# rishikksh20/FastSpeech2

Hardware: AMD Instinct MI355X
Metric: mel-frames/sec (higher is better)
Workload: dtype bf16x3 (FFN conv: f16 x f16 + block-scaled e4m3 cross terms; the decoder's: block-scaled e2m1 cross terms, one E8M0 scale per 16-channel block on both operands); 1 GPU; c3: batch=64 LJSpeech-shape; default.yaml dims, free-running, random-init weights (seed 0), duration bias calibrated to 7.87 frames/phoneme; precision=mix_mx4, utterances=64, phonemes=4528, parallelism=single GPU, launch=eager, device-driven layout (no host sync), overlap_encoder=False, streams=3

## Files before the change

fastspeech2_amd/csrc/attn_bf16.h:

```cpp
#pragma once
#include "common.h"
#include "gemm_bf16.h"

namespace fs2 {

constexpr int kAttAlign = 8;

struct QkvSplitArgs {
    const float* qkv; int R; int Rvt; int D; int dk; float scale;
    __bf16 *qk_hi, *qk_lo;
    __bf16 *vt_hi, *vt_lo;
};

__global__ __launch_bounds__(256) void qkv_split(QkvSplitArgs a) {
    extern __shared__ __attribute__((aligned(16))) float vt_s[];
    const int tid = threadIdx.x;
    const int r0 = blockIdx.x * 32;
    const int D = a.D, ld = 3 * D;
    const int groups = 2 * D / 8;
    for (int idx = tid; idx < 32 * groups; idx += 256) {
        const int r = idx / groups, c = (idx - r * groups) * 8;
        const int row = r0 + r;
        if (row >= a.R) continue;
        const float* src = a.qkv + (size_t)row * ld + c;
// ... 11 lines not shown
        const int r = idx / (D / 4), c = (idx - r * (D / 4)) * 4;
        const int row = r0 + r;
        float4 v = make_float4(0.f, 0.f, 0.f, 0.f);
        if (row < a.R) v = *reinterpret_cast<const float4*>(a.qkv + (size_t)row * ld + 2 * D + c);
        float* d = vt_s + r * ldv + c;
        d[0] = v.x; d[1] = v.y; d[2] = v.z; d[3] = v.w;
    }
    __syncthreads();
    for (int idx = tid; idx < D * 4; idx += 256) {
        const int n = idx >> 2, j = idx & 3;
        float4 p, q;
        const float* s = vt_s + (8 * j) * ldv + n;
        p.x = s[0]; p.y = s[ldv]; p.z = s[2 * ldv]; p.w = s[3 * ldv];
        q.x = s[4 * ldv]; q.y = s[5 * ldv]; q.z = s[6 * ldv]; q.w = s[7 * ldv];
        const SplitPair sp = split8(p, q);
        const size_t off = (size_t)n * a.Rvt + r0 + 8 * j;
        *reinterpret_cast<uint4*>(a.vt_hi + off) = sp.hi;
        *reinterpret_cast<uint4*>(a.vt_lo + off) = sp.lo;
    }
}

struct AttnB16Args {
    const __bf16 *qk_hi, *qk_lo; int ldqk;
    const __bf16 *vt_hi, *vt_lo; int Rvt;
    float* ctx; int ldc;
    void* ctxp; int ctxp_chunks;
    const int* start; const int* len; const int* klen;
    const int2* work;
    const int* nwork;
    int nitems;
    int D; int mask_q;
    unsigned qk_lo_bytes, vt_lo_bytes;
    int *slow_count, *slow_count2;
};

__device__ __forceinline__ float quad_rows_max(float v) {
    auto r = __builtin_amdgcn_permlane16_swap(__float_as_uint(v), __float_as_uint(v), false, false);
    v = fmaxf(__uint_as_float(r[0]), __uint_as_float(r[1]));
    r = __builtin_amdgcn_permlane32_swap(__float_as_uint(v), __float_as_uint(v), false, false);
    return fmaxf(__uint_as_float(r[0]), __uint_as_float(r[1]));
}
__device__ __forceinline__ float quad_rows_sum(float v) {
    auto r = __builtin_amdgcn_permlane16_swap(__float_as_uint(v), __float_as_uint(v), false, false);
    v = __uint_as_float(r[0]) + __uint_as_float(r[1]);
    r = __builtin_amdgcn_permlane32_swap(__float_as_uint(v), __float_as_uint(v), false, false);
    return __uint_as_float(r[0]) + __uint_as_float(r[1]);
}

template <int DK>
constexpr size_t attn_b16_lds_bytes() { return (size_t)32 * DK * 4 + (size_t)DK * 128; }

#ifdef FS2_ATT_TIMING
__device__ long long g_att_phase[8];
#define FS2_T(i) { const long long t_ = __builtin_readcyclecounter(); if (blockIdx.x == 0 && blockIdx.y == 0 && threadIdx.x == 0) g_att_phase[i] += t_ - tprev; tprev = t_; }
#else
#define FS2_T(i)
#endif

template <int DK, int NSPLIT>
__global__ __launch_bounds__(256, 2) void attn_bf16(AttnB16Args a) {
    extern __shared__ __attribute__((aligned(16))) char smem_a[];
    constexpr int KROW = DK * 4;
    constexpr int KSL = DK / 8;
    constexpr int NC = DK / 32;
    constexpr int NT = DK / 16;
    char* Ks = smem_a;
// ... 292 lines not shown
```

fastspeech2_amd/csrc/attn_w32.h:

```cpp
#pragma once
#include <type_traits>
#include <utility>
#include "attn_bf16.h"

namespace fs2 {

typedef float f32x16 __attribute__((ext_vector_type(16)));

template <int DK>
constexpr size_t attn_w32_lds_bytes() { return (size_t)3 * (32 * DK * 4 + DK * 128); }

template <class F, int... I>
__device__ __forceinline__ void for_seq(F&& f, std::integer_sequence<int, I...>) { (f(std::integral_constant<int, I>{}), ...); }

template <int N>
__device__ __forceinline__ void mfma_o0(const bf16x8_t& z_v) {
    if constexpr (N == 0) asm volatile("s_nop 3\n\tv_mfma_f32_32x32x16_bf16 a[0:15], %0, %0, 0" : : "v"(z_v) : "a0", "a1", "a2", "a3", "a4", "a5", "a6", "a7", "a8", "a9", "a10", "a11", "a12", "a13", "a14", "a15");
    else if constexpr (N == 1) asm volatile("s_nop 3\n\tv_mfma_f32_32x32x16_bf16 a[16:31], %0, %0, 0" : : "v"(z_v) : "a16", "a17", "a18", "a19", "a20", "a21", "a22", "a23", "a24", "a25", "a26", "a27", "a28", "a29", "a30", "a31");
    else if constexpr (N == 2) asm volatile("s_nop 3\n\tv_mfma_f32_32x32x16_bf16 a[32:47], %0, %0, 0" : : "v"(z_v) : "a32", "a33", "a34", "a35", "a36", "a37", "a38", "a39", "a40", "a41", "a42", "a43", "a44", "a45", "a46", "a47");
    else if constexpr (N == 3) asm volatile("s_nop 3\n\tv_mfma_f32_32x32x16_bf16 a[48:63], %0, %0, 0" : : "v"(z_v) : "a48", "a49", "a50", "a51", "a52", "a53", "a54", "a55", "a56", "a57", "a58", "a59", "a60", "a61", "a62", "a63");
    else if constexpr (N == 4) asm volatile("s_nop 3\n\tv_mfma_f32_32x32x16_bf16 a[64:79], %0, %0, 0" : : "v"(z_v) : "a64", "a65", "a66", "a67", "a68", "a69", "a70", "a71", "a72", "a73", "a74", "a75", "a76", "a77", "a78", "a79");
    else if constexpr (N == 5) asm volatile("s_nop 3\n\tv_mfma_f32_32x32x16_bf16 a[80:95], %0, %0, 0" : : "v"(z_v) : "a80", "a81", "a82", "a83", "a84", "a85", "a86", "a87", "a88", "a89", "a90", "a91", "a92", "a93", "a94", "a95");
    else if constexpr (N == 6) asm volatile("s_nop 3\n\tv_mfma_f32_32x32x16_bf16 a[96:111], %0, %0, 0" : : "v"(z_v) : "a96", "a97", "a98", "a99", "a100", "a101", "a102", "a103", "a104", "a105", "a106", "a107", "a108", "a109", "a110", "a111");
    else if constexpr (N == 7) asm volatile("s_nop 3\n\tv_mfma_f32_32x32x16_bf16 a[112:127], %0, %0, 0" : : "v"(z_v) : "a112", "a113", "a114", "a115", "a116", "a117", "a118", "a119", "a120", "a121", "a122", "a123", "a124", "a125", "a126", "a127");
}
template <int N>
__device__ __forceinline__ void read_o(float (&e)[16]) {
    if constexpr (N == 0) asm volatile("v_accvgpr_read_b32 %0, a0\n\tv_accvgpr_read_b32 %1, a1\n\tv_accvgpr_read_b32 %2, a2\n\tv_accvgpr_read_b32 %3, a3\n\tv_accvgpr_read_b32 %4, a4\n\tv_accvgpr_read_b32 %5, a5\n\tv_accvgpr_read_b32 %6, a6\n\tv_accvgpr_read_b32 %7, a7\n\tv_accvgpr_read_b32 %8, a8\n\tv_accvgpr_read_b32 %9, a9\n\tv_accvgpr_read_b32 %10, a10\n\tv_accvgpr_read_b32 %11, a11\n\tv_accvgpr_read_b32 %12, a12\n\tv_accvgpr_read_b32 %13, a13\n\tv_accvgpr_read_b32 %14, a14\n\tv_accvgpr_read_b32 %15, a15" : "=v"(e[0]), "=v"(e[1]), "=v"(e[2]), "=v"(e[3]), "=v"(e[4]), "=v"(e[5]), "=v"(e[6]), "=v"(e[7]), "=v"(e[8]), "=v"(e[9]), "=v"(e[10]), "=v"(e[11]), "=v"(e[12]), "=v"(e[13]), "=v"(e[14]), "=v"(e[15]));
    else if constexpr (N == 1) asm volatile("v_accvgpr_read_b32 %0, a16\n\tv_accvgpr_read_b32 %1, a17\n\tv_accvgpr_read_b32 %2, a18\n\tv_accvgpr_read_b32 %3, a19\n\tv_accvgpr_read_b32 %4, a20\n\tv_accvgpr_read_b32 %5, a21\n\tv_accvgpr_read_b32 %6, a22\n\tv_accvgpr_read_b32 %7, a23\n\tv_accvgpr_read_b32 %8, a24\n\tv_accvgpr_read_b32 %9, a25\n\tv_accvgpr_read_b32 %10, a26\n\tv_accvgpr_read_b32 %11, a27\n\tv_accvgpr_read_b32 %12, a28\n\tv_accvgpr_read_b32 %13, a29\n\tv_accvgpr_read_b32 %14, a30\n\tv_accvgpr_read_b32 %15, a31" : "=v"(e[0]), "=v"(e[1]), "=v"(e[2]), "=v"(e[3]), "=v"(e[4]), "=v"(e[5]), "=v"(e[6]), "=v"(e[7]), "=v"(e[8]), "=v"(e[9]), "=v"(e[10]), "=v"(e[11]), "=v"(e[12]), "=v"(e[13]), "=v"(e[14]), "=v"(e[15]));
    else if constexpr (N == 2) asm volatile("v_accvgpr_read_b32 %0, a32\n\tv_accvgpr_read_b32 %1, a33\n\tv_accvgpr_read_b32 %2, a34\n\tv_accvgpr_read_b32 %3, a35\n\tv_accvgpr_read_b32 %4, a36\n\tv_accvgpr_read_b32 %5, a37\n\tv_accvgpr_read_b32 %6, a38\n\tv_accvgpr_read_b32 %7, a39\n\tv_accvgpr_read_b32 %8, a40\n\tv_accvgpr_read_b32 %9, a41\n\tv_accvgpr_read_b32 %10, a42\n\tv_accvgpr_read_b32 %11, a43\n\tv_accvgpr_read_b32 %12, a44\n\tv_accvgpr_read_b32 %13, a45\n\tv_accvgpr_read_b32 %14, a46\n\tv_accvgpr_read_b32 %15, a47" : "=v"(e[0]), "=v"(e[1]), "=v"(e[2]), "=v"(e[3]), "=v"(e[4]), "=v"(e[5]), "=v"(e[6]), "=v"(e[7]), "=v"(e[8]), "=v"(e[9]), "=v"(e[10]), "=v"(e[11]), "=v"(e[12]), "=v"(e[13]), "=v"(e[14]), "=v"(e[15]));
    else if constexpr (N == 3) asm volatile("v_accvgpr_read_b32 %0, a48\n\tv_accvgpr_read_b32 %1, a49\n\tv_accvgpr_read_b32 %2, a50\n\tv_accvgpr_read_b32 %3, a51\n\tv_accvgpr_read_b32 %4, a52\n\tv_accvgpr_read_b32 %5, a53\n\tv_accvgpr_read_b32 %6, a54\n\tv_accvgpr_read_b32 %7, a55\n\tv_accvgpr_read_b32 %8, a56\n\tv_accvgpr_read_b32 %9, a57\n\tv_accvgpr_read_b32 %10, a58\n\tv_accvgpr_read_b32 %11, a59\n\tv_accvgpr_read_b32 %12, a60\n\tv_accvgpr_read_b32 %13, a61\n\tv_accvgpr_read_b32 %14, a62\n\tv_accvgpr_read_b32 %15, a63" : "=v"(e[0]), "=v"(e[1]), "=v"(e[2]), "=v"(e[3]), "=v"(e[4]), "=v"(e[5]), "=v"(e[6]), "=v"(e[7]), "=v"(e[8]), "=v"(e[9]), "=v"(e[10]), "=v"(e[11]), "=v"(e[12]), "=v"(e[13]), "=v"(e[14]), "=v"(e[15]));
    else if constexpr (N == 4) asm volatile("v_accvgpr_read_b32 %0, a64\n\tv_accvgpr_read_b32 %1, a65\n\tv_accvgpr_read_b32 %2, a66\n\tv_accvgpr_read_b32 %3, a67\n\tv_accvgpr_read_b32 %4, a68\n\tv_accvgpr_read_b32 %5, a69\n\tv_accvgpr_read_b32 %6, a70\n\tv_accvgpr_read_b32 %7, a71\n\tv_accvgpr_read_b32 %8, a72\n\tv_accvgpr_read_b32 %9, a73\n\tv_accvgpr_read_b32 %10, a74\n\tv_accvgpr_read_b32 %11, a75\n\tv_accvgpr_read_b32 %12, a76\n\tv_accvgpr_read_b32 %13, a77\n\tv_accvgpr_read_b32 %14, a78\n\tv_accvgpr_read_b32 %15, a79" : "=v"(e[0]), "=v"(e[1]), "=v"(e[2]), "=v"(e[3]), "=v"(e[4]), "=v"(e[5]), "=v"(e[6]), "=v"(e[7]), "=v"(e[8]), "=v"(e[9]), "=v"(e[10]), "=v"(e[11]), "=v"(e[12]), "=v"(e[13]), "=v"(e[14]), "=v"(e[15]));
    else if constexpr (N == 5) asm volatile("v_accvgpr_read_b32 %0, a80\n\tv_accvgpr_read_b32 %1, a81\n\tv_accvgpr_read_b32 %2, a82\n\tv_accvgpr_read_b32 %3, a83\n\tv_accvgpr_read_b32 %4, a84\n\tv_accvgpr_read_b32 %5, a85\n\tv_accvgpr_read_b32 %6, a86\n\tv_accvgpr_read_b32 %7, a87\n\tv_accvgpr_read_b32 %8, a88\n\tv_accvgpr_read_b32 %9, a89\n\tv_accvgpr_read_b32 %10, a90\n\tv_accvgpr_read_b32 %11, a91\n\tv_accvgpr_read_b32 %12, a92\n\tv_accvgpr_read_b32 %13, a93\n\tv_accvgpr_read_b32 %14, a94\n\tv_accvgpr_read_b32 %15, a95" : "=v"(e[0]), "=v"(e[1]), "=v"(e[2]), "=v"(e[3]), "=v"(e[4]), "=v"(e[5]), "=v"(e[6]), "=v"(e[7]), "=v"(e[8]), "=v"(e[9]), "=v"(e[10]), "=v"(e[11]), "=v"(e[12]), "=v"(e[13]), "=v"(e[14]), "=v"(e[15]));
    else if constexpr (N == 6) asm volatile("v_accvgpr_read_b32 %0, a96\n\tv_accvgpr_read_b32 %1, a97\n\tv_accvgpr_read_b32 %2, a98\n\tv_accvgpr_read_b32 %3, a99\n\tv_accvgpr_read_b32 %4, a100\n\tv_accvgpr_read_b32 %5, a101\n\tv_accvgpr_read_b32 %6, a102\n\tv_accvgpr_read_b32 %7, a103\n\tv_accvgpr_read_b32 %8, a104\n\tv_accvgpr_read_b32 %9, a105\n\tv_accvgpr_read_b32 %10, a106\n\tv_accvgpr_read_b32 %11, a107\n\tv_accvgpr_read_b32 %12, a108\n\tv_accvgpr_read_b32 %13, a109\n\tv_accvgpr_read_b32 %14, a110\n\tv_accvgpr_read_b32 %15, a111" : "=v"(e[0]), "=v"(e[1]), "=v"(e[2]), "=v"(e[3]), "=v"(e[4]), "=v"(e[5]), "=v"(e[6]), "=v"(e[7]), "=v"(e[8]), "=v"(e[9]), "=v"(e[10]), "=v"(e[11]), "=v"(e[12]), "=v"(e[13]), "=v"(e[14]), "=v"(e[15]));
    else if constexpr (N == 7) asm volatile("v_accvgpr_read_b32 %0, a112\n\tv_accvgpr_read_b32 %1, a113\n\tv_accvgpr_read_b32 %2, a114\n\tv_accvgpr_read_b32 %3, a115\n\tv_accvgpr_read_b32 %4, a116\n\tv_accvgpr_read_b32 %5, a117\n\tv_accvgpr_read_b32 %6, a118\n\tv_accvgpr_read_b32 %7, a119\n\tv_accvgpr_read_b32 %8, a120\n\tv_accvgpr_read_b32 %9, a121\n\tv_accvgpr_read_b32 %10, a122\n\tv_accvgpr_read_b32 %11, a123\n\tv_accvgpr_read_b32 %12, a124\n\tv_accvgpr_read_b32 %13, a125\n\tv_accvgpr_read_b32 %14, a126\n\tv_accvgpr_read_b32 %15, a127" : "=v"(e[0]), "=v"(e[1]), "=v"(e[2]), "=v"(e[3]), "=v"(e[4]), "=v"(e[5]), "=v"(e[6]), "=v"(e[7]), "=v"(e[8]), "=v"(e[9]), "=v"(e[10]), "=v"(e[11]), "=v"(e[12]), "=v"(e[13]), "=v"(e[14]), "=v"(e[15]));
}
template <int KIND>
__device__ __forceinline__ void mfma_s(f32x16& acc, const bf16x8_t& a_v, const bf16x8_t& b_a, const f32x16& cm) {
    if constexpr (KIND == 1) asm volatile("v_mfma_f32_32x32x16_bf16 %0, %1, %2, %3" : "=&v"(acc) : "v"(a_v), "a"(b_a), "v"(cm));
    else if constexpr (KIND == 2) asm volatile("v_mfma_f32_32x32x16_bf16 %0, %1, %2, 0" : "=&v"(acc) : "v"(a_v), "a"(b_a));
    else asm volatile("v_mfma_f32_32x32x16_bf16 %0, %1, %2, %0" : "+v"(acc) : "v"(a_v), "a"(b_a));
}
template <int N, bool PAD>
// ... 78 lines not shown
        const float p = __builtin_amdgcn_exp2f(score(key) - m);
        l += p;
#pragma unroll
        for (int c = 0; c < NC; ++c) acc[c] = fmaf(p, (float)vh[(size_t)c * a.Rvt + key] + (float)vl[(size_t)c * a.Rvt + key], acc[c]);
    }
    const float linv = (l > 0.f) ? 1.f / l : 0.f;
    const bool dead = a.mask_q && qrow >= klen;
    const size_t row = (size_t)(s0 + qrow);
#pragma unroll
    for (int c = 0; c < NC; c += 4) {
        const int col = h * DK + hi * NC + c;
        f32x4 v = f32x4{acc[c], acc[c + 1], acc[c + 2], acc[c + 3]} * linv;
        if (dead) v = f32x4{0.f, 0.f, 0.f, 0.f};
        if (a.ctx) *reinterpret_cast<f32x4*>(a.ctx + row * a.ldc + col) = v;
        if (a.ctxp) store_planes4(a.ctxp, row, a.ctxp_chunks, col, v);
    }
}

template <int DK>
__global__ __launch_bounds__(256, 1) void attn_w32(AttnB16Args a) {
    static_assert(DK % 64 == 0 && DK <= 256, "head dim: a multiple of 64 up to 256");
    extern __shared__ __attribute__((aligned(16))) char smem_w[];
    constexpr int KSL = DK / 8;
    constexpr int KROWB = DK * 4;
    constexpr int KB = 32 * KROWB;
    constexpr int VB = DK * 128;
    constexpr int NKS = DK / 16;
    constexpr int NT = DK / 32;
    constexpr int PW = DK / 32;
    using I0 = std::integral_constant<int, 0>;
    using I1 = std::integral_constant<int, 1>;
    const int tid = threadIdx.x, lane = tid & 63;
#ifdef FS2_W32_TIMING
    long long wstamp[12] = {0, 0, 0, 0, 0, 0, 0, 0, 0, 0, 0, 0};
    long long tpro = __builtin_readcyclecounter();
#define FS2_WP(i) { const long long t_ = __builtin_readcyclecounter(); wstamp[i] += t_ - tpro; tpro = t_; }
#else
#define FS2_WP(i)
#endif
    const int wave = __builtin_amdgcn_readfirstlane(tid >> 6);
    const int l31 = lane & 31, hi = lane >> 5;
    {
        const int nitems = a.nwork != nullptr ? *a.nwork : a.nitems;
        if ((int)blockIdx.x >= nitems) return;
    }
    const int2 wk = a.work[blockIdx.x];
    const int b = __builtin_amdgcn_readfirstlane(wk.x), h = blockIdx.y;
    if (b < 0) return;
    const int s0 = __builtin_amdgcn_readfirstlane(a.start[b]), len = __builtin_amdgcn_readfirstlane(a.len[b]);
    const int klen = __builtin_amdgcn_readfirstlane(a.klen[b]);
    const int q0 = __builtin_amdgcn_readfirstlane(wk.y) * kAttBlk + wave * 32;
    const bool wave_live = q0 < len;
    const int ntiles = (klen + 31) >> 5;
    const unsigned lds0 = __builtin_amdgcn_readfirstlane((unsigned)(size_t)(lds_void_t*)smem_w);
    FS2_WP(8)

    auto k_piece = [&](int u, int ln, int& key, int& byte_in_row) __attribute__((always_inline)) {
        const int G = (u * 4 + wave) * 64 + ln;
        const int rho = G / (2 * KSL), ps = G - rho * (2 * KSL);
        const int s = (ps & ~15) | ((ps & 15) ^ (rho & 15));
        const int plane = s >= KSL;
        key = (rho & 19) | ((rho & 4) << 1) | ((rho & 8) >> 1);
        byte_in_row = (s - plane * KSL) * 16 + plane * (int)a.qk_lo_bytes;
    };
    auto v_piece = [&](int u, int ln, int& n, int& j, int& plane) __attribute__((always_inline)) {
        const int G = (u * 4 + wave) * 64 + ln;
        n = G >> 3;
        const int s = (G & 7) ^ ((n >> 1) & 7);
        j = s & 3; plane = s >> 2;
    };
    unsigned kgo[PW], vgo[PW];
#pragma unroll
    for (int u = 0; u < PW; ++u) {
        int key, bir, n, j, plane;
        k_piece(u, lane, key, bir);
        kgo[u] = (unsigned)(key * a.ldqk * 2 + bir);
        v_piece(u, lane, n, j, plane);
        vgo[u] = (unsigned)n * (unsigned)a.Rvt * 2u + (unsigned)j * 16u + (unsigned)plane * a.vt_lo_bytes;
    }
    gchar_t* kbase = uniform_ptr(reinterpret_cast<const char*>(a.qk_hi + a.D + (size_t)h * DK) + (size_t)s0 * a.ldqk * 2);
    gchar_t* vbase = uniform_ptr(reinterpret_cast<const char*>(a.vt_hi + (size_t)h * DK * a.Rvt + s0));

    auto issue_K = [&](int kt, int buf) __attribute__((always_inline)) {
        const int key0 = kt * 32;
        const unsigned dst = lds0 + buf * KB + wave * 1024;
        if (key0 + 32 <= klen) {
            gchar_t* base = uniform_ptr((const void*)(kbase + (size_t)key0 * a.ldqk * 2));
            asm volatile("s_nop 4" ::: "memory");
#pragma unroll
            for (int u = 0; u < PW; ++u) dma16_so(base, kgo[u], dst + u * 4096);
        } else {
            int ln = lane;
            asm volatile("" : "+v"(ln));
#pragma unroll
            for (int u = 0; u < PW; ++u) {
                int key, bir;
                k_piece(u, ln, key, bir);
                dma16((const void*)(kbase + (size_t)min(key0 + key, klen - 1) * a.ldqk * 2 + bir), dst + u * 4096);
            }
        }
    };
    auto issue_V = [&](int kt, int buf) __attribute__((always_inline)) {
        const int key0 = kt * 32;
        const unsigned dst = lds0 + 3 * KB + buf * VB + wave * 1024;
        gchar_t* base = uniform_ptr((const void*)(vbase + (size_t)key0 * 2));
        if (key0 + 32 <= klen) {
            asm volatile("s_nop 4" ::: "memory");
#pragma unroll
            for (int u = 0; u < PW; ++u) dma16_so(base, vgo[u], dst + u * 4096);
        } else {
            int ln = lane;
            asm volatile("" : "+v"(ln));
#pragma unroll
            for (int u = 0; u < PW; ++u) {
                int n, j, plane;
                v_piece(u, ln, n, j, plane);
                const int nv = klen - (key0 + 8 * j);
                const unsigned go = (unsigned)n * (unsigned)a.Rvt * 2u + (unsigned)j * 16u + (unsigned)plane * a.vt_lo_bytes;
                const void* sp = (nv > 0) ? (const void*)(base + go) : static_cast<const void*>(g_zero16);
                dma16(sp, dst + u * 4096);
            }
        }
    };
    auto fix_V = [&](int kt, int buf) __attribute__((always_inline)) {
        const int key0 = kt * 32;
        if (key0 + 32 <= klen || (klen & 7) == 0) return;
        int ln = lane;
        asm volatile("" : "+v"(ln));
#pragma unroll
        for (int u = 0; u < PW; ++u) {
            int n, j, plane;
            v_piece(u, ln, n, j, plane);
            const int nv = klen - (key0 + 8 * j);
            if (nv > 0 && nv < 8) {
                u32x4* p = reinterpret_cast<u32x4*>(smem_w + 3 * KB + buf * VB + (u * 4 + wave) * 1024 + ln * 16);
                u32x4 v = *p;
#pragma unroll
                for (int w = 0; w < 4; ++w) v[w] &= (nv > 2 * w + 1) ? 0xffffffffu : ((nv > 2 * w) ? 0x0000ffffu : 0u);
                *p = v;
            }
        }
    };

    const char* kp[8];
    {
        const int g = hi ^ (l31 & 15);
#pragma unroll
        for (int e = 0; e < 8; ++e) kp[e] = smem_w + l31 * KROWB + ((((2 * e) ^ (g & 14)) | (g & 1)) << 4);
    }
    const char* vp[4];
    {
        const int g = hi ^ ((l31 >> 1) & 7);
#pragma unroll
        for (int e = 0; e < 4; ++e) vp[e] = smem_w + 3 * KB + l31 * 128 + ((((2 * e) ^ (g & 6)) | (g & 1)) << 4);
    }

    FS2_WP(9)
    if (ntiles > 0) issue_K(0, 0);
    static_assert(KB == VB, "the Q staging region spans K and V^T ring slots of equal size");
    bf16x8_t qh[NKS], ql[NKS];
    {
        gchar_t* qbase = (gchar_t*)reinterpret_cast<const char*>(a.qk_hi + (size_t)h * DK);
#pragma unroll
        for (int pc = 0; pc < KSL; ++pc) {
            const int G = pc * 64 + lane;
            const int rho = G / (2 * KSL), ps = G - rho * (2 * KSL);
            const int sl = (ps & ~15) | ((ps & 15) ^ (rho & 15));
            const int plane = sl >= KSL;
            const int qr = min(q0 + rho, len - 1);
            dma16((const void*)(qbase + (size_t)(s0 + qr) * a.ldqk * 2 + (sl - plane * KSL) * 16 + (size_t)plane * a.qk_lo_bytes), lds0 + (1 + wave) * KB + pc * 1024);
        }
        asm volatile("s_waitcnt vmcnt(0)" ::: "memory");
        const int qoff = (1 + wave) * KB;
#pragma unroll
        for (int c = 0; c < NKS; ++c) {
            const int sh = 2 * c, sl = KSL + 2 * c;
            qh[c] = *reinterpret_cast<const bf16x8_t*>(kp[(sh & 15) >> 1] + qoff + (sh >> 4) * 256);
            ql[c] = *reinterpret_cast<const bf16x8_t*>(kp[(sl & 15) >> 1] + qoff + (sl >> 4) * 256);
            asm volatile("" : "+a"(qh[c]), "+a"(ql[c]));
        }
    }
    FS2_WP(10)
    {
        const bf16x8_t z = __builtin_bit_cast(bf16x8_t, u32x4{0, 0, 0, 0});
        for_seq([&](auto n_tag) __attribute__((always_inline)) { mfma_o0<decltype(n_tag)::value>(z); }, std::make_integer_sequence<int, NT>{});
    }
    float l_run = 0.f;
    int bail = 0;
    f32x16 am, ac;
    f32x16 negm;
    float p[16];
    unsigned phw[8], plw[8];
    float psum, psum_row = 0.f;
    typedef __bf16 bf16x2_t __attribute__((ext_vector_type(2)));
    typedef float f32x2_t __attribute__((ext_vector_type(2)));
    auto pack2 = [&](float x, float y) __attribute__((always_inline)) {
        return __builtin_bit_cast(unsigned, __builtin_convertvector(f32x2_t{x, y}, bf16x2_t));
    };

    constexpr int kTailSteps = 34;
    auto tail_step = [&](auto t_tag) __attribute__((always_inline)) {
        constexpr int T = decltype(t_tag)::value;
        if constexpr (T < 32) {
            constexpr int J = T >> 2, U = T & 3, R = 2 * J;
            if constexpr (U == 0) {
                if constexpr (J == 0) psum = 0.f;
                asm volatile("v_exp_f32 %0, %0\n\tv_exp_f32 %1, %1\n\ts_nop 0" : "+v"(p[R]), "+v"(p[R + 1]));
            } else if constexpr (U == 1) {
                psum += p[R];
                psum += p[R + 1];
                phw[J] = pack2(p[R], p[R + 1]);
                asm volatile("" : "+v"(phw[J]));
            } else if constexpr (U == 2) {
                p[R] -= __uint_as_float(phw[J] << 16);
                p[R + 1] -= __uint_as_float(phw[J] & 0xffff0000u);
            } else {
                plw[J] = pack2(p[R], p[R + 1]);
                asm volatile("" : "+v"(plw[J]));
            }
// ... 114 lines not shown
                int key, bir;
                k_piece(u, ln, key, bir);
                koff[u] = (unsigned)((min(kk * 32 + key, klen - 1) - kk * 32) * a.ldqk * 2 + bir);
            }
        }
        if (kv >= 0) {
            gchar_t* base = vbase + (size_t)kv * 64;
#pragma unroll
            for (int u = 0; u < PW; ++u) vptr[u] = base + vgo[u];
            if (kv * 32 + 32 > klen) {
                int ln = lane;
                asm volatile("" : "+v"(ln));
#pragma unroll
                for (int u = 0; u < PW; ++u) {
                    int n, j, plane;
                    v_piece(u, ln, n, j, plane);
                    if (klen - (kv * 32 + 8 * j) <= 0) vptr[u] = (gchar_t*)reinterpret_cast<const char*>(g_zero16);
                }
            }
        }
    };

    auto tile = [&](auto r_tag, int kt) __attribute__((always_inline)) {
        constexpr int R = decltype(r_tag)::value;
        using IV = std::integral_constant<int, R>;
        using IK = std::integral_constant<int, (R + 1) % 3>;
        constexpr int KD = R, VD = (R + 2) % 3;
        const bool has_next = kt + 1 < ntiles;
        const int dk = min(kt + 3, ntiles - 1), dv = min(kt + 2, ntiles - 1);
#ifdef FS2_W32_TIMING
        long long tprev = __builtin_readcyclecounter();
        wstamp[4] += 1;
#endif
        if (wave_live && !bail) {
            if (has_next) {
                prep_dma(dk, dv);
                gchar_t* kb = uniform_ptr((const void*)(kbase + (size_t)dk * 32 * a.ldqk * 2));
                asm volatile("s_nop 4" ::: "memory");
                const unsigned kdst = lds0 + KD * KB + wave * 1024, vdst = lds0 + 3 * KB + VD * VB + wave * 1024;
                if ((kt + 1) * 32 + 32 <= klen) {
                    phase_a(IK{}, I1{}, kb, kdst);
                    FS2_WT(0)
                    phase_b(IV{}, I1{}, I1{}, vdst);
                } else {
                    phase_a(IK{}, I1{}, kb, kdst);
                    FS2_WT(0)
                    phase_b(IV{}, I0{}, I1{}, vdst);
                    for_seq([&](auto t_tag) __attribute__((always_inline)) { head_step(t_tag, I1{}, (kt + 1) * 32); }, std::make_integer_sequence<int, kHeadSteps>{});
                }
            } else {
                for_seq(tail_step, std::make_integer_sequence<int, kTailSteps>{});
                phase_b(IV{}, I0{}, I0{}, 0u);
            }
            bail = __builtin_amdgcn_readfirstlane(__any(!(psum_row < kW32SumLimit)));
            if (FS2_W32_ABL & 250) bail = 0;
        } else if (has_next) {
            issue_K(dk, KD);
            issue_V(dv, VD);
        }
        FS2_WT(1)
        if (has_next && !(FS2_W32_ABL & 4)) {
            if constexpr (FS2_W32_ABL & 16) {}
            else if constexpr (2 * PW == 12) asm volatile("s_waitcnt vmcnt(12)" ::: "memory");
            else if constexpr (2 * PW == 8) asm volatile("s_waitcnt vmcnt(8)" ::: "memory");
            else if constexpr (2 * PW == 4) asm volatile("s_waitcnt vmcnt(4)" ::: "memory");
            else asm volatile("s_waitcnt vmcnt(0)" ::: "memory");
            FS2_WT(2)
            if (kt + 2 == ntiles) fix_V(kt + 1, (R + 1) % 3);
            if constexpr (!(FS2_W32_ABL & 32)) __syncthreads();
            FS2_WT(3)
        }
    };

    if (ntiles > 0) {
        asm volatile("s_waitcnt vmcnt(0)" ::: "memory");
        __syncthreads();
        FS2_WP(5)
        issue_K(min(1, ntiles - 1), 1);
        issue_K(min(2, ntiles - 1), 2);
        issue_V(0, 0);
        issue_V(min(1, ntiles - 1), 1);
        if (wave_live) {
            phase_a(I0{}, I0{}, kbase, 0u);
            mfma_drain();
            if (32 <= klen) for_seq([&](auto t_tag) __attribute__((always_inline)) { head_step(t_tag, I0{}, 0); }, std::make_integer_sequence<int, kHeadSteps>{});
            else for_seq([&](auto t_tag) __attribute__((always_inline)) { head_step(t_tag, I1{}, 0); }, std::make_integer_sequence<int, kHeadSteps>{});
            const float m0 = row_max();
#pragma unroll
            for (int r = 0; r < 16; ++r) { p[r] -= m0; negm[r] = -m0; }
        }
        asm volatile("s_waitcnt vmcnt(0)" ::: "memory");
#pragma unroll
        for (int c = 0; c < NKS; ++c) asm volatile("" : : "a"(qh[c]), "a"(ql[c]));
        if (ntiles == 1) fix_V(0, 0);
        __syncthreads();
        FS2_WP(6)
        for (int kt = 0; kt < ntiles; kt += 3) {
            tile(I0{}, kt);
            if (kt + 1 < ntiles) tile(I1{}, kt + 1);
            if (kt + 2 < ntiles) tile(std::integral_constant<int, 2>{}, kt + 2);
        }
    }
#ifdef FS2_W32_TIMING
    tpro = __builtin_readcyclecounter();
#endif
    const bool staged = a.ctxp != nullptr && a.ctx == nullptr;
    if (staged) {
        asm volatile("s_waitcnt vmcnt(0)" ::: "memory");
        __syncthreads();
    }
    if (!wave_live) return;
    if (bail) {
        attn_w32_rows_slow<DK>(a, s0, len, klen, q0, h, lane);
        return;
    }

    mfma_drain();
    const int qrow = q0 + l31;
    const float linv = (l_run > 0.f) ? 1.f / l_run : 0.f;
    const bool dead = a.mask_q && qrow >= klen;
    if (staged) {
        constexpr int RS = DK * 4 + 16;
        char* stage = smem_w + wave * (32 * RS);
        for_seq([&](auto n_tag) __attribute__((always_inline)) {
            constexpr int nt = decltype(n_tag)::value;
            float e[16];
            read_o<nt>(e);
#pragma unroll
            for (int g = 0; g < 4; ++g) {
                f32x4 v = f32x4{e[4 * g], e[4 * g + 1], e[4 * g + 2], e[4 * g + 3]} * linv;
                if (dead) v = f32x4{0.f, 0.f, 0.f, 0.f};
                uint2 vh, vl;
                split4(v, vh, vl);
                char* d = stage + l31 * RS + nt * 128 + 16 * (2 * (g & 1) + hi) + 8 * (g >> 1);
                *reinterpret_cast<uint2*>(d) = vh;
                *reinterpret_cast<uint2*>(d + 64) = vl;
            }
        }, std::make_integer_sequence<int, NT>{});
        constexpr int UPR = DK * 4 / 16;
        char* out = reinterpret_cast<char*>(a.ctxp) + ((size_t)(s0 + q0) * a.ctxp_chunks + (size_t)h * NT) * 128;
        const size_t row_bytes = (size_t)a.ctxp_chunks * 128;
#pragma unroll
        for (int i = 0; i < 32 * UPR / 64; ++i) {
            const int U = i * 64 + lane, r = U / UPR, ps = U - r * UPR;
            const u32x4 w = *reinterpret_cast<const u32x4*>(stage + r * RS + ps * 16);
            if (q0 + r < len) *reinterpret_cast<u32x4*>(out + (size_t)r * row_bytes + ps * 16) = w;
        }
    } else {
        if (qrow >= len) return;
        const size_t row = (size_t)(s0 + qrow);
        for_seq([&](auto n_tag) __attribute__((always_inline)) {
            constexpr int nt = decltype(n_tag)::value;
            float e[16];
            read_o<nt>(e);
#pragma unroll
            for (int g = 0; g < 4; ++g) {
                const int col = h * DK + 32 * nt + 8 * g + 4 * hi;
                f32x4 v = f32x4{e[4 * g], e[4 * g + 1], e[4 * g + 2], e[4 * g + 3]} * linv;
                if (dead) v = f32x4{0.f, 0.f, 0.f, 0.f};
                if (a.ctx) *reinterpret_cast<f32x4*>(a.ctx + row * a.ldc + col) = v;
                if (a.ctxp) store_planes4(a.ctxp, row, a.ctxp_chunks, col, v);
            }
        }, std::make_integer_sequence<int, NT>{});
    }
#ifdef FS2_W32_TIMING
    asm volatile("s_waitcnt vmcnt(0)" ::: "memory");
    {
        const long long t_ = __builtin_readcyclecounter();
        wstamp[7] = t_ - tpro;
        if (blockIdx.x == 0 && blockIdx.y == 0 && threadIdx.x == 0)
            for (int i = 0; i < 12; ++i) g_w32_phase[i] += wstamp[i];
    }
#endif
}

}
```

fastspeech2_amd/csrc/common.h:

```cpp
#pragma once
#include <hip/hip_runtime.h>
#include <stdint.h>

namespace fs2 {

typedef float f32x4 __attribute__((ext_vector_type(4)));
typedef unsigned int u32x4 __attribute__((ext_vector_type(4)));
typedef short bf16x8 __attribute__((ext_vector_type(8)));

constexpr int kGap = 8;
constexpr int kTailRows = 8;
constexpr int kMinGap = 4;
constexpr int kMaxHalo = 16;
constexpr int kBK = 32;
constexpr int kLd = kBK + 4;

constexpr int kAttBQ = 64;
constexpr int kAttBlk = 128;

inline unsigned att_grid64(int nitems) { return 2u * (unsigned)((nitems + 7) & ~7); }
__device__ __forceinline__ bool att_item64(const int2* work, const int* nwork, int nitems, int& b, int& q0) {
    const int x = (int)blockIdx.x;
    const int item = ((x >> 4) << 3) | (x & 7);
    if (item >= (nwork != nullptr ? *nwork : nitems)) return false;
    const int2 wk = work[item];
    b = __builtin_amdgcn_readfirstlane(wk.x);
    q0 = __builtin_amdgcn_readfirstlane(wk.y) * kAttBlk + ((x >> 3) & 1) * kAttBQ;
    return b >= 0;
}

struct SeqMeta {
    const int* start;
    const int* len;
    const int* klen;
    const int* vlen;
    const int* row_pos;
    const int* row_seq;
    int B, R;
};

struct GemmArgs {
    const float* X; int ldx; int C;
    const float* W; int Cpad; int ktaps;
    int N; int R;
    const int* row_pos;
    const float* bias;
    const float* resid; int ldr;
    int relu_pre;
    const float* ln_g; const float* ln_b; float ln_eps;
// ... 184 lines not shown
```

fastspeech2_amd/csrc/fs2_runtime.hip:

```cpp
#include <hip/hip_runtime.h>
#include <dlfcn.h>

#include <algorithm>
#include <cmath>
#include <cstdarg>
#include <cstdio>
#include <cstring>
#include <fstream>
#include <iterator>
#include <map>
#include <string>
#include <type_traits>
#include <vector>

#include "../../include/fs2.h"
#include "attn_bf16.h"
#include "attn_w32.h"
#include "attn_f32.h"
#include "common.h"
#include "elementwise.h"
#include "gemm_bf16.h"
#include "gemm_planes.h"
#include "gemm_row4.h"
#include "gemm_mx.h"
// ... 14 lines not shown
    int kw = 0;
    void* wm4 = nullptr;
    unsigned char* ws4 = nullptr;
    float* bias = nullptr;
    int N = 0, C = 0, Cpad = 0, ktaps = 1;
};
struct Layer {
    Gemm qkv, out, w1, w2;
    Gemm cat_x, cat_a;
    float *ln1g = nullptr, *ln1b = nullptr, *ln2g = nullptr, *ln2b = nullptr;
    int ka = 0;
    int kh = 0;
};
struct Predictor {
    std::vector<Gemm> conv;
    std::vector<float*> lng, lnb;
    float *lin_w = nullptr, *lin_b = nullptr;
};
struct FusedPredictors {
    bool ok = false;
    Gemm c0, c1;
    float *ln0g = nullptr, *ln0b = nullptr, *ln1g = nullptr, *ln1b = nullptr, *lin_w = nullptr, *lin_b = nullptr;
};
struct Stack {
    std::vector<Layer> layers;
    float* pe = nullptr; int pe_rows = 0;
    float* alpha = nullptr;
    int dk = 0, Dp = 0;
    bool pre_ln = false, concat = false;
    float *after_g = nullptr, *after_b = nullptr;
};

constexpr int kSplitRegime = 8192, kSplitRows = 16384;
constexpr int kXcds = 8;

struct Options {
    int bm = -1;
    int bal = 0;
    int row8 = -1;
    int qkv8 = -1;
    int nosplitk = 0;
    int f32_rows = 0;
    int fuse_var = 1;
    int mt8 = -1;
    int op_att_planes = 0;
    int qkv_split = -1;
    int w32 = -1;
    int row4 = -1;
    int mt4 = -1;
    int qkv4 = -1;
    int ffn2_mx = 1;
    int post_mx = 1;
};
int env_int(const char* name, int dflt) {
    const char* e = getenv(name);
    return e ? atoi(e) : dflt;
}

struct Sha256 {
    uint32_t h[8] = {0x6a09e667u, 0xbb67ae85u, 0x3c6ef372u, 0xa54ff53au, 0x510e527fu, 0x9b05688cu, 0x1f83d9abu, 0x5be0cd19u};
    unsigned char buf[64]; size_t fill = 0; uint64_t total = 0;
    static uint32_t rotr(uint32_t x, int n) { return (x >> n) | (x << (32 - n)); }
    void block(const unsigned char* p) {
        static const uint32_t K[64] = {
            0x428a2f98u, 0x71374491u, 0xb5c0fbcfu, 0xe9b5dba5u, 0x3956c25bu, 0x59f111f1u, 0x923f82a4u, 0xab1c5ed5u, 0xd807aa98u, 0x12835b01u, 0x243185beu, 0x550c7dc3u,
            0x72be5d74u, 0x80deb1feu, 0x9bdc06a7u, 0xc19bf174u, 0xe49b69c1u, 0xefbe4786u, 0x0fc19dc6u, 0x240ca1ccu, 0x2de92c6fu, 0x4a7484aau, 0x5cb0a9dcu, 0x76f988dau,
            0x983e5152u, 0xa831c66du, 0xb00327c8u, 0xbf597fc7u, 0xc6e00bf3u, 0xd5a79147u, 0x06ca6351u, 0x14292967u, 0x27b70a85u, 0x2e1b2138u, 0x4d2c6dfcu, 0x53380d13u,
// ... 2274 lines not shown
```

Before: 9.636 million mel-frames/s.

## Add persistent work-claiming loop to w32 attention with next-item Q/K prefetch

Restructures the w32 attention kernel so a block can loop over work items. Items are claimed from per-XCD atomic counters, and the next item's Q rows and first K tile are prefetched into spare ring slots while the current item's last tiles run. The staged output path moves to a dedicated swizzled LDS region that is written per head-tile with wave barriers, which drops the block-wide sync and full memory wait that were needed before staging. The persistent mode only turns on when a counter pointer is supplied, and the runtime shown does not set one. The non-persistent path still picks up the new prefetch, loop and staging structure, at the cost of extra LDS and more complex control flow.

```diff
diff --git a/fastspeech2_amd/csrc/attn_bf16.h b/fastspeech2_amd/csrc/attn_bf16.h
--- a/fastspeech2_amd/csrc/attn_bf16.h
+++ b/fastspeech2_amd/csrc/attn_bf16.h
@@ -67,6 +67,7 @@
     int D; int mask_q;
     unsigned qk_lo_bytes, vt_lo_bytes;
     int *slow_count, *slow_count2;
+    int* pctr = nullptr; int heads = 1;
 };
 
 __device__ __forceinline__ float quad_rows_max(float v) {
diff --git a/fastspeech2_amd/csrc/attn_w32.h b/fastspeech2_amd/csrc/attn_w32.h
--- a/fastspeech2_amd/csrc/attn_w32.h
+++ b/fastspeech2_amd/csrc/attn_w32.h
@@ -8,7 +8,7 @@
 typedef float f32x16 __attribute__((ext_vector_type(16)));
 
 template <int DK>
-constexpr size_t attn_w32_lds_bytes() { return (size_t)3 * (32 * DK * 4 + DK * 128); }
+constexpr size_t attn_w32_lds_bytes() { return (size_t)3 * (32 * DK * 4 + DK * 128) + 4 * 4096; }
 
 template <class F, int... I>
 __device__ __forceinline__ void for_seq(F&& f, std::integer_sequence<int, I...>) { (f(std::integral_constant<int, I>{}), ...); }
@@ -153,27 +153,83 @@
     using I1 = std::integral_constant<int, 1>;
     const int tid = threadIdx.x, lane = tid & 63;
 #ifdef FS2_W32_TIMING
-    long long wstamp[12] = {0, 0, 0, 0, 0, 0, 0, 0, 0, 0, 0, 0};
-    long long tpro = __builtin_readcyclecounter();
+    long long wstamp[16] = {0, 0, 0, 0, 0, 0, 0, 0, 0, 0, 0, 0, 0, 0, 0, 0};
+    long long tpro = __builtin_readcyclecounter(), tswitch = 0;
 #define FS2_WP(i) { const long long t_ = __builtin_readcyclecounter(); wstamp[i] += t_ - tpro; tpro = t_; }
 #else
 #define FS2_WP(i)
 #endif
     const int wave = __builtin_amdgcn_readfirstlane(tid >> 6);
     const int l31 = lane & 31, hi = lane >> 5;
+    const int nitems = __builtin_amdgcn_readfirstlane(a.nwork != nullptr ? *a.nwork : a.nitems);
+    const bool persist = a.pctr != nullptr;
+    if (!persist && (int)blockIdx.x >= nitems) return;
+    const unsigned lds0 = __builtin_amdgcn_readfirstlane((unsigned)(size_t)(lds_void_t*)smem_w);
+    constexpr int RING = 6 * KB;
+    int h = 0, s0 = 0, len = 0, klen = 0, q0 = 0, ntiles = 0;
+    bool wave_live = false;
+    gchar_t *kbase = nullptr, *vbase = nullptr;
+    unsigned qoff = 0;
+    int n_valid = 0, n_h = 0, n_s0 = 0, n_len = 0, n_klen = 0, n_qb = 0;
+    unsigned n_qoff = 0;
+    int* const bcast = reinterpret_cast<int*>(smem_w + RING);
+    auto claim = [&](int slot) __attribute__((always_inline)) {
+        const int j = blockIdx.x & (kXcds - 1);
+        const int total = ((nitems + kXcds - 1 - j) / kXcds) * a.heads;
+        int v = 0, ch = 0, cs = 0, cl = 0, ck = 0, cq = 0;
+        for (;;) {
+            int pr = 0;
+            if (lane == 0) pr = atomicAdd(a.pctr + j, 1);
+            pr = __builtin_amdgcn_readfirstlane(pr);
+            if (pr >= total) break;
+            const int i = pr / a.heads;
+            const int2 wk = a.work[i * kXcds + j];
+            const int b = __builtin_amdgcn_readfirstlane(wk.x);
+            if (b < 0) continue;
+            v = 1; ch = pr - i * a.heads; cq = __builtin_amdgcn_readfirstlane(wk.y);
+            cs = __builtin_amdgcn_readfirstlane(a.start[b]); cl = __builtin_amdgcn_readfirstlane(a.len[b]); ck = __builtin_amdgcn_readfirstlane(a.klen[b]);
+            break;
+        }
+        if (lane == 0) {
+            int* w = bcast + 8 * slot;
+            w[0] = v; w[1] = ch; w[2] = cs; w[3] = cl; w[4] = ck; w[5] = cq;
+        }
+    };
+    auto claimed = [&](int slot, int& v, int& ch, int& cs, int& cl, int& ck, int& cq) __attribute__((always_inline)) {
+        const int* w = bcast + 8 * slot;
+        v = __builtin_amdgcn_readfirstlane(w[0]); ch = __builtin_amdgcn_readfirstlane(w[1]); cs = __builtin_amdgcn_readfirstlane(w[2]);
+        cl = __builtin_amdgcn_readfirstlane(w[3]); ck = __builtin_amdgcn_readfirstlane(w[4]); cq = __builtin_amdgcn_readfirstlane(w[5]);
+    };
+    auto leave = [&]() __attribute__((always_inline)) {
+        if (persist && tid == 0 && atomicAdd(a.pctr + kXcds, 1) == (int)gridDim.x - 1) {
+#pragma unroll
+            for (int j = 0; j <= kXcds; ++j) a.pctr[j] = 0;
+        }
+    };
+    auto set_item = [&](int ch, int cs, int cl, int ck, int cq) __attribute__((always_inline)) {
+        h = ch; s0 = cs; len = cl; klen = ck;
+        q0 = cq * kAttBlk + wave * 32;
+        wave_live = q0 < len;
+        ntiles = (klen + 31) >> 5;
+        kbase = uniform_ptr(reinterpret_cast<const char*>(a.qk_hi + a.D + (size_t)h * DK) + (size_t)s0 * a.ldqk * 2);
+        vbase = uniform_ptr(reinterpret_cast<const char*>(a.vt_hi + (size_t)h * DK * a.Rvt + s0));
+    };
     {
-        const int nitems = a.nwork != nullptr ? *a.nwork : a.nitems;
-        if ((int)blockIdx.x >= nitems) return;
-    }
-    const int2 wk = a.work[blockIdx.x];
-    const int b = __builtin_amdgcn_readfirstlane(wk.x), h = blockIdx.y;
-    if (b < 0) return;
-    const int s0 = __builtin_amdgcn_readfirstlane(a.start[b]), len = __builtin_amdgcn_readfirstlane(a.len[b]);
-    const int klen = __builtin_amdgcn_readfirstlane(a.klen[b]);
-    const int q0 = __builtin_amdgcn_readfirstlane(wk.y) * kAttBlk + wave * 32;
-    const bool wave_live = q0 < len;
-    const int ntiles = (klen + 31) >> 5;
-    const unsigned lds0 = __builtin_amdgcn_readfirstlane((unsigned)(size_t)(lds_void_t*)smem_w);
+        int cv, ch, cs, cl, ck, cq;
+        if (persist) {
+            if (wave == 0) { claim(1); claim(0); }
+            __syncthreads();
+            claimed(1, cv, ch, cs, cl, ck, cq);
+            if (!cv) { leave(); return; }
+        } else {
+            const int2 wk = a.work[blockIdx.x];
+            const int b = __builtin_amdgcn_readfirstlane(wk.x);
+            if (b < 0) return;
+            ch = blockIdx.y; cq = __builtin_amdgcn_readfirstlane(wk.y);
+            cs = __builtin_amdgcn_readfirstlane(a.start[b]); cl = __builtin_amdgcn_readfirstlane(a.len[b]); ck = __builtin_amdgcn_readfirstlane(a.klen[b]);
+        }
+        set_item(ch, cs, cl, ck, cq);
+    }
     FS2_WP(8)
 
     auto k_piece = [&](int u, int ln, int& key, int& byte_in_row) __attribute__((always_inline)) {
@@ -199,10 +255,8 @@
         v_piece(u, lane, n, j, plane);
         vgo[u] = (unsigned)n * (unsigned)a.Rvt * 2u + (unsigned)j * 16u + (unsigned)plane * a.vt_lo_bytes;
     }
-    gchar_t* kbase = uniform_ptr(reinterpret_cast<const char*>(a.qk_hi + a.D + (size_t)h * DK) + (size_t)s0 * a.ldqk * 2);
-    gchar_t* vbase = uniform_ptr(reinterpret_cast<const char*>(a.vt_hi + (size_t)h * DK * a.Rvt + s0));
-
-    auto issue_K = [&](int kt, int buf) __attribute__((always_inline)) {
+
+    auto issue_K_of = [&](gchar_t* kbase, int klen, int kt, int buf) __attribute__((always_inline)) {
         const int key0 = kt * 32;
         const unsigned dst = lds0 + buf * KB + wave * 1024;
         if (key0 + 32 <= klen) {
@@ -221,6 +275,7 @@
             }
         }
     };
+    auto issue_K = [&](int kt, int buf) __attribute__((always_inline)) { issue_K_of(kbase, klen, kt, buf); };
     auto issue_V = [&](int kt, int buf) __attribute__((always_inline)) {
         const int key0 = kt * 32;
         const unsigned dst = lds0 + 3 * KB + buf * VB + wave * 1024;
@@ -276,36 +331,37 @@
         for (int e = 0; e < 4; ++e) vp[e] = smem_w + 3 * KB + l31 * 128 + ((((2 * e) ^ (g & 6)) | (g & 1)) << 4);
     }
 
+    static_assert(KB == VB, "the Q staging region spans K and V^T ring slots of equal size");
+    static_assert(DK == 192 || 64 % (2 * KSL) == 0 || (2 * KSL) % 64 == 0, "Q pieces: rows per piece");
+    constexpr int QPER = DK == 192 ? 3 : 1, QRP = QPER * 64 / (2 * KSL), NQC = KSL / 2;
+    unsigned qcol[NQC];
+    int qrho[QPER];
+#pragma unroll
+    for (int pc = 0; pc < NQC; ++pc) {
+        const int G = pc * 64 + lane;
+        const int rho = G / (2 * KSL), ps = G - rho * (2 * KSL);
+        const int sl = (ps & ~15) | ((ps & 15) ^ (rho & 15));
+        const int plane = sl >= KSL;
+        qcol[pc] = (unsigned)((sl - plane * KSL) * 16) + (unsigned)plane * a.qk_lo_bytes;
+        if (pc < QPER) qrho[pc] = rho;
+    }
+    auto q_slot = [&](int vl) __attribute__((always_inline)) { return (unsigned)((wave < 2 ? 1 + wave : 3 + (vl + wave - 1) % 3) * KB); };
+    auto prefetch = [&](int ph, int ps0, int plen, int pklen, int pq0, unsigned qo) __attribute__((always_inline)) {
+        if (pklen > 0) issue_K_of(uniform_ptr(reinterpret_cast<const char*>(a.qk_hi + a.D + (size_t)ph * DK) + (size_t)ps0 * a.ldqk * 2), pklen, 0, 0);
+        gchar_t* qb = uniform_ptr(reinterpret_cast<const char*>(a.qk_hi + (size_t)ph * DK) + (size_t)ps0 * a.ldqk * 2);
+        asm volatile("s_nop 4" ::: "memory");
+        const unsigned ld2 = (unsigned)a.ldqk * 2u;
+#pragma unroll
+        for (int pc = 0; pc < KSL; ++pc) {
+            const int qr = min(pq0 + QRP * (pc / QPER) + qrho[pc % QPER], plen - 1);
+            dma16_so(qb, (unsigned)qr * ld2 + qcol[pc % NQC], lds0 + qo + pc * 1024);
+        }
+    };
     FS2_WP(9)
-    if (ntiles > 0) issue_K(0, 0);
-    static_assert(KB == VB, "the Q staging region spans K and V^T ring slots of equal size");
+    qoff = q_slot(2);
+    prefetch(h, s0, len, klen, q0, qoff);
+    FS2_WP(10)
     bf16x8_t qh[NKS], ql[NKS];
-    {
-        gchar_t* qbase = (gchar_t*)reinterpret_cast<const char*>(a.qk_hi + (size_t)h * DK);
-#pragma unroll
-        for (int pc = 0; pc < KSL; ++pc) {
-            const int G = pc * 64 + lane;
-            const int rho = G / (2 * KSL), ps = G - rho * (2 * KSL);
-            const int sl = (ps & ~15) | ((ps & 15) ^ (rho & 15));
-            const int plane = sl >= KSL;
-            const int qr = min(q0 + rho, len - 1);
-            dma16((const void*)(qbase + (size_t)(s0 + qr) * a.ldqk * 2 + (sl - plane * KSL) * 16 + (size_t)plane * a.qk_lo_bytes), lds0 + (1 + wave) * KB + pc * 1024);
-        }
-        asm volatile("s_waitcnt vmcnt(0)" ::: "memory");
-        const int qoff = (1 + wave) * KB;
-#pragma unroll
-        for (int c = 0; c < NKS; ++c) {
-            const int sh = 2 * c, sl = KSL + 2 * c;
-            qh[c] = *reinterpret_cast<const bf16x8_t*>(kp[(sh & 15) >> 1] + qoff + (sh >> 4) * 256);
-            ql[c] = *reinterpret_cast<const bf16x8_t*>(kp[(sl & 15) >> 1] + qoff + (sl >> 4) * 256);
-            asm volatile("" : "+a"(qh[c]), "+a"(ql[c]));
-        }
-    }
-    FS2_WP(10)
-    {
-        const bf16x8_t z = __builtin_bit_cast(bf16x8_t, u32x4{0, 0, 0, 0});
-        for_seq([&](auto n_tag) __attribute__((always_inline)) { mfma_o0<decltype(n_tag)::value>(z); }, std::make_integer_sequence<int, NT>{});
-    }
     float l_run = 0.f;
     int bail = 0;
     f32x16 am, ac;
@@ -486,6 +542,11 @@
         long long tprev = __builtin_readcyclecounter();
         wstamp[4] += 1;
 #endif
+        if (!has_next && n_valid) {
+            n_qoff = q_slot(R);
+            prefetch(n_h, n_s0, n_len, n_klen, n_qb * kAttBlk + wave * 32, n_qoff);
+        }
+        FS2_WT(15)
         if (wave_live && !bail) {
             if (has_next) {
                 prep_dma(dk, dv);
@@ -515,6 +576,7 @@
         FS2_WT(1)
         if (has_next && !(FS2_W32_ABL & 4)) {
             if constexpr (FS2_W32_ABL & 16) {}
+            else if (kt + 2 == ntiles) asm volatile("s_waitcnt vmcnt(0)" ::: "memory");
             else if constexpr (2 * PW == 12) asm volatile("s_waitcnt vmcnt(12)" ::: "memory");
             else if constexpr (2 * PW == 8) asm volatile("s_waitcnt vmcnt(8)" ::: "memory");
             else if constexpr (2 * PW == 4) asm volatile("s_waitcnt vmcnt(4)" ::: "memory");
@@ -526,105 +588,133 @@
         }
     };
 
-    if (ntiles > 0) {
+    for (;;) {
+        FS2_WP(14)
         asm volatile("s_waitcnt vmcnt(0)" ::: "memory");
+#pragma unroll
+        for (int c = 0; c < NKS; ++c) {
+            const int sh = 2 * c, sl = KSL + 2 * c;
+            qh[c] = *reinterpret_cast<const bf16x8_t*>(kp[(sh & 15) >> 1] + qoff + (sh >> 4) * 256);
+            ql[c] = *reinterpret_cast<const bf16x8_t*>(kp[(sl & 15) >> 1] + qoff + (sl >> 4) * 256);
+            asm volatile("" : "+a"(qh[c]), "+a"(ql[c]));
+        }
         __syncthreads();
+        if (persist) {
+            claimed(0, n_valid, n_h, n_s0, n_len, n_klen, n_qb);
+            if (ntiles == 0) __syncthreads();
+        }
         FS2_WP(5)
-        issue_K(min(1, ntiles - 1), 1);
-        issue_K(min(2, ntiles - 1), 2);
-        issue_V(0, 0);
-        issue_V(min(1, ntiles - 1), 1);
+        {
+            const bf16x8_t z = __builtin_bit_cast(bf16x8_t, u32x4{0, 0, 0, 0});
+            for_seq([&](auto n_tag) __attribute__((always_inline)) { mfma_o0<decltype(n_tag)::value>(z); }, std::make_integer_sequence<int, NT>{});
+        }
+        l_run = 0.f; bail = 0; psum_row = 0.f;
+        if (ntiles > 0) {
+            issue_K(min(1, ntiles - 1), 1);
+            issue_K(min(2, ntiles - 1), 2);
+            issue_V(0, 0);
+            issue_V(min(1, ntiles - 1), 1);
+#ifdef FS2_W32_TIMING
+            if (tswitch) { wstamp[11] += __builtin_readcyclecounter() - tswitch; wstamp[12] += 1; }
+#endif
+            if (wave_live) {
+                phase_a(I0{}, I0{}, kbase, 0u);
+                mfma_drain();
+                if (32 <= klen) for_seq([&](auto t_tag) __attribute__((always_inline)) { head_step(t_tag, I0{}, 0); }, std::make_integer_sequence<int, kHeadSteps>{});
+                else for_seq([&](auto t_tag) __attribute__((always_inline)) { head_step(t_tag, I1{}, 0); }, std::make_integer_sequence<int, kHeadSteps>{});
+                const float m0 = row_max();
+#pragma unroll
+                for (int r = 0; r < 16; ++r) { p[r] -= m0; negm[r] = -m0; }
+            }
+            asm volatile("s_waitcnt vmcnt(0)" ::: "memory");
+#pragma unroll
+            for (int c = 0; c < NKS; ++c) asm volatile("" : : "a"(qh[c]), "a"(ql[c]));
+            if (ntiles == 1) fix_V(0, 0);
+            __syncthreads();
+            FS2_WP(6)
+            for (int kt = 0; kt < ntiles; kt += 3) {
+                tile(I0{}, kt);
+                if (kt + 1 < ntiles) tile(I1{}, kt + 1);
+                if (kt + 2 < ntiles) tile(std::integral_constant<int, 2>{}, kt + 2);
+            }
+        } else if (n_valid) {
+            n_qoff = q_slot(2);
+            prefetch(n_h, n_s0, n_len, n_klen, n_qb * kAttBlk + wave * 32, n_qoff);
+        }
+#ifdef FS2_W32_TIMING
+        tpro = __builtin_readcyclecounter();
+        tswitch = tpro;
+        wstamp[13] += 1;
+#endif
         if (wave_live) {
-            phase_a(I0{}, I0{}, kbase, 0u);
-            mfma_drain();
-            if (32 <= klen) for_seq([&](auto t_tag) __attribute__((always_inline)) { head_step(t_tag, I0{}, 0); }, std::make_integer_sequence<int, kHeadSteps>{});
-            else for_seq([&](auto t_tag) __attribute__((always_inline)) { head_step(t_tag, I1{}, 0); }, std::make_integer_sequence<int, kHeadSteps>{});
-            const float m0 = row_max();
-#pragma unroll
-            for (int r = 0; r < 16; ++r) { p[r] -= m0; negm[r] = -m0; }
-        }
-        asm volatile("s_waitcnt vmcnt(0)" ::: "memory");
-#pragma unroll
-        for (int c = 0; c < NKS; ++c) asm volatile("" : : "a"(qh[c]), "a"(ql[c]));
-        if (ntiles == 1) fix_V(0, 0);
-        __syncthreads();
-        FS2_WP(6)
-        for (int kt = 0; kt < ntiles; kt += 3) {
-            tile(I0{}, kt);
-            if (kt + 1 < ntiles) tile(I1{}, kt + 1);
-            if (kt + 2 < ntiles) tile(std::integral_constant<int, 2>{}, kt + 2);
-        }
-    }
-#ifdef FS2_W32_TIMING
-    tpro = __builtin_readcyclecounter();
-#endif
-    const bool staged = a.ctxp != nullptr && a.ctx == nullptr;
-    if (staged) {
-        asm volatile("s_waitcnt vmcnt(0)" ::: "memory");
-        __syncthreads();
-    }
-    if (!wave_live) return;
-    if (bail) {
-        attn_w32_rows_slow<DK>(a, s0, len, klen, q0, h, lane);
-        return;
-    }
-
-    mfma_drain();
-    const int qrow = q0 + l31;
-    const float linv = (l_run > 0.f) ? 1.f / l_run : 0.f;
-    const bool dead = a.mask_q && qrow >= klen;
-    if (staged) {
-        constexpr int RS = DK * 4 + 16;
-        char* stage = smem_w + wave * (32 * RS);
-        for_seq([&](auto n_tag) __attribute__((always_inline)) {
-            constexpr int nt = decltype(n_tag)::value;
-            float e[16];
-            read_o<nt>(e);
-#pragma unroll
-            for (int g = 0; g < 4; ++g) {
-                f32x4 v = f32x4{e[4 * g], e[4 * g + 1], e[4 * g + 2], e[4 * g + 3]} * linv;
-                if (dead) v = f32x4{0.f, 0.f, 0.f, 0.f};
-                uint2 vh, vl;
-                split4(v, vh, vl);
-                char* d = stage + l31 * RS + nt * 128 + 16 * (2 * (g & 1) + hi) + 8 * (g >> 1);
-                *reinterpret_cast<uint2*>(d) = vh;
-                *reinterpret_cast<uint2*>(d + 64) = vl;
-            }
-        }, std::make_integer_sequence<int, NT>{});
-        constexpr int UPR = DK * 4 / 16;
-        char* out = reinterpret_cast<char*>(a.ctxp) + ((size_t)(s0 + q0) * a.ctxp_chunks + (size_t)h * NT) * 128;
-        const size_t row_bytes = (size_t)a.ctxp_chunks * 128;
-#pragma unroll
-        for (int i = 0; i < 32 * UPR / 64; ++i) {
-            const int U = i * 64 + lane, r = U / UPR, ps = U - r * UPR;
-            const u32x4 w = *reinterpret_cast<const u32x4*>(stage + r * RS + ps * 16);
-            if (q0 + r < len) *reinterpret_cast<u32x4*>(out + (size_t)r * row_bytes + ps * 16) = w;
-        }
-    } else {
-        if (qrow >= len) return;
-        const size_t row = (size_t)(s0 + qrow);
-        for_seq([&](auto n_tag) __attribute__((always_inline)) {
-            constexpr int nt = decltype(n_tag)::value;
-            float e[16];
-            read_o<nt>(e);
-#pragma unroll
-            for (int g = 0; g < 4; ++g) {
-                const int col = h * DK + 32 * nt + 8 * g + 4 * hi;
-                f32x4 v = f32x4{e[4 * g], e[4 * g + 1], e[4 * g + 2], e[4 * g + 3]} * linv;
-                if (dead) v = f32x4{0.f, 0.f, 0.f, 0.f};
-                if (a.ctx) *reinterpret_cast<f32x4*>(a.ctx + row * a.ldc + col) = v;
-                if (a.ctxp) store_planes4(a.ctxp, row, a.ctxp_chunks, col, v);
-            }
-        }, std::make_integer_sequence<int, NT>{});
-    }
+            if (bail) {
+                attn_w32_rows_slow<DK>(a, s0, len, klen, q0, h, lane);
+            } else {
+                mfma_drain();
+                int ln = lane;
+                asm volatile("" : "+v"(ln));
+                const int l31 = ln & 31, hi = ln >> 5, lane = ln;
+                const int qrow = q0 + l31;
+                const float linv = (l_run > 0.f) ? 1.f / l_run : 0.f;
+                const bool dead = a.mask_q && qrow >= klen;
+                if (a.ctxp != nullptr && a.ctx == nullptr) {
+                    char* stage = smem_w + RING + wave * 4096;
+                    char* out = reinterpret_cast<char*>(a.ctxp) + ((size_t)(s0 + q0) * a.ctxp_chunks + (size_t)h * NT) * 128;
+                    const size_t row_bytes = (size_t)a.ctxp_chunks * 128;
+                    for_seq([&](auto n_tag) __attribute__((always_inline)) {
+                        constexpr int nt = decltype(n_tag)::value;
+                        float e[16];
+                        read_o<nt>(e);
+#pragma unroll
+                        for (int g = 0; g < 4; ++g) {
+                            f32x4 v = f32x4{e[4 * g], e[4 * g + 1], e[4 * g + 2], e[4 * g + 3]} * linv;
+                            if (dead) v = f32x4{0.f, 0.f, 0.f, 0.f};
+                            uint2 vh, vl;
+                            split4(v, vh, vl);
+                            const int u = 2 * (g & 1) + hi;
+                            char* d = stage + l31 * 128 + 8 * (g >> 1);
+                            *reinterpret_cast<uint2*>(d + ((u ^ (l31 & 7)) << 4)) = vh;
+                            *reinterpret_cast<uint2*>(d + (((u + 4) ^ (l31 & 7)) << 4)) = vl;
+                        }
+                        __builtin_amdgcn_wave_barrier();
+#pragma unroll
+                        for (int i = 0; i < 4; ++i) {
+                            const int U = i * 64 + lane, r = U >> 3, ps = U & 7;
+                            const u32x4 w = *reinterpret_cast<const u32x4*>(stage + r * 128 + ((ps ^ (r & 7)) << 4));
+                            if (q0 + r < len) *reinterpret_cast<u32x4*>(out + (size_t)r * row_bytes + nt * 128 + ps * 16) = w;
+                        }
+                        __builtin_amdgcn_wave_barrier();
+                    }, std::make_integer_sequence<int, NT>{});
+                } else if (qrow < len) {
+                    const size_t row = (size_t)(s0 + qrow);
+                    for_seq([&](auto n_tag) __attribute__((always_inline)) {
+                        constexpr int nt = decltype(n_tag)::value;
+                        float e[16];
+                        read_o<nt>(e);
+#pragma unroll
+                        for (int g = 0; g < 4; ++g) {
+                            const int col = h * DK + 32 * nt + 8 * g + 4 * hi;
+                            f32x4 v = f32x4{e[4 * g], e[4 * g + 1], e[4 * g + 2], e[4 * g + 3]} * linv;
+                            if (dead) v = f32x4{0.f, 0.f, 0.f, 0.f};
+                            if (a.ctx) *reinterpret_cast<f32x4*>(a.ctx + row * a.ldc + col) = v;
+                            if (a.ctxp) store_planes4(a.ctxp, row, a.ctxp_chunks, col, v);
+                        }
+                    }, std::make_integer_sequence<int, NT>{});
+                }
+            }
+        }
+        FS2_WP(7)
+        if (!n_valid) break;
+        if (wave == 0) claim(0);
+        set_item(n_h, n_s0, n_len, n_klen, n_qb);
+        qoff = n_qoff;
+        n_valid = 0;
+    }
+    leave();
 #ifdef FS2_W32_TIMING
     asm volatile("s_waitcnt vmcnt(0)" ::: "memory");
-    {
-        const long long t_ = __builtin_readcyclecounter();
-        wstamp[7] = t_ - tpro;
-        if (blockIdx.x == 0 && blockIdx.y == 0 && threadIdx.x == 0)
-            for (int i = 0; i < 12; ++i) g_w32_phase[i] += wstamp[i];
-    }
+    if (blockIdx.x == 0 && blockIdx.y == 0 && threadIdx.x == 0)
+        for (int i = 0; i < 16; ++i) g_w32_phase[i] += wstamp[i];
 #endif
 }
 
diff --git a/fastspeech2_amd/csrc/common.h b/fastspeech2_amd/csrc/common.h
--- a/fastspeech2_amd/csrc/common.h
+++ b/fastspeech2_amd/csrc/common.h
@@ -15,6 +15,7 @@
 constexpr int kBK = 32;
 constexpr int kLd = kBK + 4;
 
+constexpr int kXcds = 8;
 constexpr int kAttBQ = 64;
 constexpr int kAttBlk = 128;
 
diff --git a/fastspeech2_amd/csrc/fs2_runtime.hip b/fastspeech2_amd/csrc/fs2_runtime.hip
--- a/fastspeech2_amd/csrc/fs2_runtime.hip
+++ b/fastspeech2_amd/csrc/fs2_runtime.hip
@@ -70,7 +70,6 @@
 };
 
 constexpr int kSplitRegime = 8192, kSplitRows = 16384;
-constexpr int kXcds = 8;
 
 struct Options {
     int bm = -1;
```

Result: no change. 9.609 million mel-frames/s (median of 2 runs) (-0.3%).
